# yuz1wan/unified_video_action

Measured on AMD Instinct MI355X. Metric: train samples/sec (video+action step) at 1/2/4/8 MI355X; loss parity, higher is better.
Workload: dtype bf16; 1 GPU; pusht_video: PushT video_model (BASELINE configs[1]); step = frame select+resize -> KL-VAE encode (8 frames) -> mar_base MAR fwd/bwd (N=1024) -> diffusion loss -> backward -> fused AdamW + EMA -> LR step; dropout 0.1; model=UVA mar_base + KL-VAE f16, global_batch=32, seq_len=1024, parallelism=dp1

## Files before the change

unified_video_action_amd/csrc/attention.hip:

```cpp
#include "attention_frag.h"

#define ATT_PRIO_HI() __builtin_amdgcn_s_setprio(1)
#define ATT_PRIO_LO() __builtin_amdgcn_s_setprio(0)
#define AT_LD 80
#define AT_TILE (64 * AT_LD)

__device__ __forceinline__ void stage_load(const bf16* __restrict__ g, long long ld, int row0, bf16x8 (&r)[2]) {
  const int t = threadIdx.x;
  const bf16* base = g + (long long)row0 * ld;
#pragma unroll
  for (int i = 0; i < 2; ++i) {
    const int id = t + i * 256, row = id >> 3, c = (id & 7) * 8;
    r[i] = *(const bf16x8*)(base + (long long)row * ld + c);
  }
}
__device__ __forceinline__ void stage_store(bf16* lds, const bf16x8 (&r)[2]) {
  const int t = threadIdx.x;
#pragma unroll
  for (int i = 0; i < 2; ++i) {
    int id = t + i * 256, row = id >> 3, c = (id & 7) * 8;
    *(bf16x8*)(lds + row * AT_LD + c) = r[i];
  }
}

__device__ __forceinline__ float keep_bfe(float v, uint32_t w, int b) {
  int m;
  asm("v_bfe_i32 %0, %1, %2, 1" : "=v"(m) : "v"(w), "s"(b));
  return __int_as_float(__float_as_int(v) & m);
}
__device__ __forceinline__ float fmax_nc(float a, float b) { return __builtin_amdgcn_fmed3f(a, b, INFINITY); }

constexpr int MASK_TPW = 4;
__device__ __forceinline__ uint32_t shift_in_sign(uint32_t acc, uint32_t t) {
  return __builtin_amdgcn_alignbit(acc, t, 31);
}
__global__ __launch_bounds__(256) void attn_mask_kernel(uint64_t* __restrict__ MQ, uint64_t* __restrict__ MK, int N,
                                                        int nt, long long waves, uint32_t th, uint64_t seed) {
  const long long wv = __builtin_amdgcn_readfirstlane((int)(blockIdx.x * 4u + (threadIdx.x >> 6)));
  if (wv >= waves) return;
  const int L = threadIdx.x & 63;
  const int per_row = (nt + MASK_TPW - 1) / MASK_TPW;
  const int kv0 = (int)(wv % per_row) * MASK_TPW;
  const long long t2 = wv / per_row;
  const int qb = (int)(t2 % nt);
  const long long bh = t2 / nt;
  const int q = qb * 64 + mask_pos(L);
  const uint32_t key = drop_key(seed);
  const uint64_t rowpair = (((uint64_t)bh * N + q) * (uint64_t)N) >> 1;
#pragma unroll 1
  for (int kv = kv0; kv < kv0 + MASK_TPW && kv < nt; ++kv) {
    const uint32_t x0 = drop_first(key, rowpair + (uint64_t)kv * 32);
    uint32_t lo = 0, hi = 0;
#pragma unroll
    for (int P = 31; P >= 0; --P) {
      const uint32_t x = drop_mix(x0 ^ (uint32_t)(mask_pos(2 * P) >> 1));
      const uint32_t t0 = (x & 0xFFFFu) - th, t1 = (x >> 16) - th;
      if (P >= 16) {
        hi = shift_in_sign(shift_in_sign(hi, t1), t0);
      } else {
        lo = shift_in_sign(shift_in_sign(lo, t1), t0);
      }
    }
    lo = ~lo;
    hi = ~hi;
    MQ[((long long)bh * nt + kv) * N + q] = ((uint64_t)hi << 32) | lo;
    {
      const bool up = L & 32;
      const auto r = __builtin_amdgcn_permlane32_swap(up ? lo : hi, up ? lo : hi, false, false);
      const uint32_t o = up ? r[0] : r[1];
      if (up) lo = o; else hi = o;
    }
#define UVA_TSTAGE(J, M)                                                                    \
  {                                                                                         \
    const bool up = L & (J);                                                                \
    const uint32_t sr = up ? 0u : (uint32_t)(J);  \
    const uint32_t km = up ? ~(M) : (M);                                                    \
    const uint32_t rl = (uint32_t)__builtin_amdgcn_ds_swizzle((int)((lo >> sr) & (M)), 0x1F | ((J) << 10)); \
    const uint32_t rh = (uint32_t)__builtin_amdgcn_ds_swizzle((int)((hi >> sr) & (M)), 0x1F | ((J) << 10)); \
    lo = (lo & km) | (rl << sr);                                                            \
    hi = (hi & km) | (rh << sr);                                                            \
  }
    UVA_TSTAGE(16, 0x0000FFFFu)
    UVA_TSTAGE(8, 0x00FF00FFu)
    UVA_TSTAGE(4, 0x0F0F0F0Fu)
    UVA_TSTAGE(2, 0x33333333u)
    UVA_TSTAGE(1, 0x55555555u)
#undef UVA_TSTAGE
    MK[((long long)bh * nt + qb) * N + (long long)kv * 64 + mask_pos(L)] = ((uint64_t)hi << 32) | lo;
  }
}

template <bool DROP, int KT, int OCC>
__global__ __launch_bounds__(256, OCC) void attn_fwd_kernel(const bf16* __restrict__ qkv, bf16* __restrict__ out,
                                                       float* __restrict__ lse2, const uint64_t* __restrict__ MQ,
                                                       int N, int H, float c, float dsc) {
  constexpr int NKT = KT / 16;
  constexpr int NH = KT / 64;
  __shared__ __attribute__((aligned(16))) bf16 sK[2][NH * AT_TILE];
  __shared__ __attribute__((aligned(16))) bf16 sV[2][NH * AT_TILE];
  int bx, bh;
  xcd_grid2(bx, bh);
  const int b = bh / H, h = bh % H;
  const long long ld = 3LL * H * 64;
  const bf16* Qg = qkv + (long long)b * N * ld + h * 64;
  const bf16* Kg = Qg + H * 64;
  const bf16* Vg = Qg + 2 * H * 64;
  const int w = threadIdx.x >> 6, l = threadIdx.x & 63, g = l >> 4, li = l & 15;
  const int q0 = bx * 128 + w * 32;
  const int nkv = N / KT, n64 = N / 64;
  const uint16_t* mq = DROP ? (const uint16_t*)(MQ + (long long)bh * n64 * N) : nullptr;

  bf16x8 qf[2][2];
  uint32_t mw[2][NH], mwn[2][NH];
#pragma unroll
  for (int qt = 0; qt < 2; ++qt) {
    const int row = q0 + qt * 16 + li;
#pragma unroll
    for (int ks = 0; ks < 2; ++ks)
      qf[qt][ks] = row < N ? *(const bf16x8*)(Qg + (long long)row * ld + ks * 32 + 8 * g) : (bf16x8){};
#pragma unroll
    for (int hh = 0; hh < NH; ++hh) {
      mw[qt][hh] = (DROP && row < N) ? mq[((long long)hh * N + row) * 4 + g] : 0u;
      mwn[qt][hh] = 0u;
    }
  }
  float m[2] = {-INFINITY, -INFINITY}, rs[2] = {0.f, 0.f};
  f32x4 o[2][4];
#pragma unroll
  for (int qt = 0; qt < 2; ++qt)
#pragma unroll
    for (int dt = 0; dt < 4; ++dt) o[qt][dt] = (f32x4){0.f, 0.f, 0.f, 0.f};

  bf16x8 rk[NH][2], rv[NH][2];
#pragma unroll
  for (int hh = 0; hh < NH; ++hh) {
    stage_load(Kg, ld, hh * 64, rk[hh]);
    stage_load(Vg, ld, hh * 64, rv[hh]);
  }
#pragma unroll
  for (int hh = 0; hh < NH; ++hh) {
    stage_store(sK[0] + hh * AT_TILE, rk[hh]);
    stage_store(sV[0] + hh * AT_TILE, rv[hh]);
  }
  __syncthreads();
  int cur = 0;
  for (int kv = 0; kv < nkv; ++kv) {
    const bool more = kv + 1 < nkv;
    if (more) {
#pragma unroll
      for (int hh = 0; hh < NH; ++hh) {
        stage_load(Kg, ld, (kv + 1) * KT + hh * 64, rk[hh]);
        stage_load(Vg, ld, (kv + 1) * KT + hh * 64, rv[hh]);
      }
      if (DROP) {
#pragma unroll
        for (int qt = 0; qt < 2; ++qt) {
          const int row = q0 + qt * 16 + li;
#pragma unroll
          for (int hh = 0; hh < NH; ++hh)
            mwn[qt][hh] = row < N ? mq[((long long)((kv + 1) * NH + hh) * N + row) * 4 + g] : 0u;
        }
      }
    }
    const bf16* cK = sK[cur];
    const bf16* cV = sV[cur];
    f32x4 s[NKT][2];
#pragma unroll
    for (int kt = 0; kt < NKT; ++kt)
#pragma unroll
      for (int qt = 0; qt < 2; ++qt) s[kt][qt] = (f32x4){0.f, 0.f, 0.f, 0.f};
    ATT_PRIO_HI();
#pragma unroll
    for (int ks = 0; ks < 2; ++ks) {
#pragma unroll
      for (int kt = 0; kt < NKT; ++kt) {
        const bf16x8 kf = row_frag<AT_LD>(cK, kt * 16, ks);
#pragma unroll
        for (int qt = 0; qt < 2; ++qt) s[kt][qt] = mfma16(kf, qf[qt][ks], s[kt][qt]);
      }
    }
    ATT_PRIO_LO();
    float mx[2];
    bool need = false;
#pragma unroll
    for (int qt = 0; qt < 2; ++qt) {
      float a = fmax_nc(s[0][qt][0], s[0][qt][1]);
#pragma unroll
      for (int kt = 0; kt < NKT; ++kt)
#pragma unroll
        for (int r = (kt == 0 ? 2 : 0); r < 4; ++r) a = fmax_nc(a, s[kt][qt][r]);
      a = quad_max(a);
      mx[qt] = a * c;
      need |= mx[qt] > m[qt] + 8.0f;
    }
    if (__builtin_amdgcn_ballot_w64(need)) {
#pragma unroll
      for (int qt = 0; qt < 2; ++qt) {
        const float mnew = fmaxf(m[qt], mx[qt]);
        const float alpha = exp2_fast(m[qt] - mnew);
        rs[qt] *= alpha;
#pragma unroll
        for (int dt = 0; dt < 4; ++dt) o[qt][dt] *= alpha;
        m[qt] = mnew;
      }
    }
#pragma unroll
    for (int qt = 0; qt < 2; ++qt) {
      const float nm = -m[qt];
      float ps[4] = {0.f, 0.f, 0.f, 0.f};
#pragma unroll
      for (int kt = 0; kt < NKT; ++kt)
#pragma unroll
        for (int r = 0; r < 4; ++r) {
          const float p = exp2_fast(fmaf(s[kt][qt][r], c, nm));
          ps[r] += p;
          s[kt][qt][r] = DROP ? keep_bfe(p, mw[qt][kt >> 2], (kt & 3) * 4 + r) : p;
        }
      rs[qt] += (ps[0] + ps[1]) + (ps[2] + ps[3]);
    }
    ATT_PRIO_HI();
#pragma unroll
    for (int ks = 0; ks < KT / 32; ++ks) {
      bf16x8 pf[2];
#pragma unroll
      for (int qt = 0; qt < 2; ++qt) pf[qt] = pack_pi(s[2 * ks][qt], s[2 * ks + 1][qt]);
#pragma unroll
      for (int dt = 0; dt < 4; ++dt) {
        const bf16x8 vf = tr_frag<AT_LD>(cV, 32 * ks, 32 * ks + 16, dt * 16);
#pragma unroll
        for (int qt = 0; qt < 2; ++qt) o[qt][dt] = mfma16(vf, pf[qt], o[qt][dt]);
      }
    }
    ATT_PRIO_LO();
    if (more) {
#pragma unroll
      for (int hh = 0; hh < NH; ++hh) {
        stage_store(sK[cur ^ 1] + hh * AT_TILE, rk[hh]);
        stage_store(sV[cur ^ 1] + hh * AT_TILE, rv[hh]);
      }
      if (DROP) {
#pragma unroll
        for (int qt = 0; qt < 2; ++qt)
#pragma unroll
          for (int hh = 0; hh < NH; ++hh) mw[qt][hh] = mwn[qt][hh];
      }
    }
    __syncthreads();
    cur ^= 1;
  }
  const long long ldo = (long long)H * 64;
#pragma unroll
  for (int qt = 0; qt < 2; ++qt) {
    float lsum = rs[qt];
    lsum += __shfl_xor(lsum, 16, 64);
    lsum += __shfl_xor(lsum, 32, 64);
    const int q = q0 + qt * 16 + li;
    if (q >= N) continue;
    const float inv = dsc / lsum;
    bf16* orow = out + ((long long)b * N + q) * ldo + h * 64;
#pragma unroll
    for (int dt = 0; dt < 4; ++dt) {
      bf16x4 v = {(bf16)(o[qt][dt][0] * inv), (bf16)(o[qt][dt][1] * inv), (bf16)(o[qt][dt][2] * inv),
                  (bf16)(o[qt][dt][3] * inv)};
      *(bf16x4*)(orow + dt * 16 + 4 * g) = v;
    }
    if (g == 0) lse2[(long long)bh * N + q] = m[qt] + __log2f(lsum);
  }
}

template <bool DROP>
__global__ __launch_bounds__(256, 2) void attn_bwd_dkdv_kernel(const bf16* __restrict__ qkv,
                                                               const bf16* __restrict__ dOs,
                                                               const float* __restrict__ lse2,
                                                               const float* __restrict__ Dvec,
                                                               const uint64_t* __restrict__ MK, bf16* __restrict__ dqkv,
                                                               int N, int H, float scale, float c, float vsc,
                                                               float* __restrict__ cpart) {
  __shared__ __attribute__((aligned(16))) bf16 sQ[2][AT_TILE];
  __shared__ __attribute__((aligned(16))) bf16 sO[2][AT_TILE];
  __shared__ __attribute__((aligned(16))) float sL[2][64];
  __shared__ __attribute__((aligned(16))) float sD[2][64];
  int bx, bh;
  xcd_grid2(bx, bh);
  const int b = bh / H, h = bh % H;
  const long long ld = 3LL * H * 64, ldo = (long long)H * 64;
  const bf16* Qg = qkv + (long long)b * N * ld + h * 64;
  const bf16* Kg = Qg + H * 64;
  const bf16* Vg = Qg + 2 * H * 64;
  const bf16* dOg = dOs + (long long)b * N * ldo + h * 64;
  const float* Lg = lse2 + (long long)bh * N;
  const float* Dg = Dvec + (long long)bh * N;
  const int w = threadIdx.x >> 6, l = threadIdx.x & 63, g = l >> 4, li = l & 15;
  const int k0 = bx * 128 + w * 32;
  const int nq = N / 64;
  const uint16_t* mk = DROP ? (const uint16_t*)(MK + (long long)bh * nq * N) : nullptr;

  bf16x8 kf[2][2], vf[2][2];
  uint32_t mw[2] = {0u, 0u}, mwn[2] = {0u, 0u};
#pragma unroll
  for (int kt = 0; kt < 2; ++kt) {
    const int row = k0 + kt * 16 + li;
    const bool ok = row < N;
#pragma unroll
    for (int ks = 0; ks < 2; ++ks) {
      kf[kt][ks] = ok ? *(const bf16x8*)(Kg + (long long)row * ld + ks * 32 + 8 * g) : (bf16x8){};
      vf[kt][ks] = ok ? *(const bf16x8*)(Vg + (long long)row * ld + ks * 32 + 8 * g) : (bf16x8){};
    }
    if (DROP) mw[kt] = ok ? mk[(long long)row * 4 + g] : 0u;
  }
  f32x4 dv[4][2], dk[4][2];
#pragma unroll
  for (int dt = 0; dt < 4; ++dt)
#pragma unroll
    for (int kt = 0; kt < 2; ++kt) dv[dt][kt] = dk[dt][kt] = (f32x4){0.f, 0.f, 0.f, 0.f};

  bf16x8 rq[2], ro[2];
  stage_load(Qg, ld, 0, rq);
  stage_load(dOg, ldo, 0, ro);
  stage_store(sQ[0], rq);
  stage_store(sO[0], ro);
  if (threadIdx.x < 64) { sL[0][threadIdx.x] = Lg[threadIdx.x]; sD[0][threadIdx.x] = Dg[threadIdx.x]; }
  __syncthreads();
  int cur = 0;
  for (int qi = 0; qi < nq; ++qi) {
    const bool more = qi + 1 < nq;
    float nl = 0.f, nd = 0.f;
    if (more) {
      stage_load(Qg, ld, (qi + 1) * 64, rq);
      stage_load(dOg, ldo, (qi + 1) * 64, ro);
      if (threadIdx.x < 64) { nl = Lg[(qi + 1) * 64 + threadIdx.x]; nd = Dg[(qi + 1) * 64 + threadIdx.x]; }
      if (DROP) {
#pragma unroll
        for (int kt = 0; kt < 2; ++kt) {
          const int row = k0 + kt * 16 + li;
          mwn[kt] = row < N ? mk[((long long)(qi + 1) * N + row) * 4 + g] : 0u;
        }
      }
    }
    f32x4 s[4][2], dp[4][2];
#pragma unroll
    for (int qt = 0; qt < 4; ++qt)
#pragma unroll
      for (int kt = 0; kt < 2; ++kt) s[qt][kt] = dp[qt][kt] = (f32x4){0.f, 0.f, 0.f, 0.f};
#pragma unroll
    for (int ks = 0; ks < 2; ++ks)
#pragma unroll
      for (int qt = 0; qt < 4; ++qt) {
        bf16x8 a = row_frag<AT_LD>(sQ[cur], qt * 16, ks);
        bf16x8 e = row_frag<AT_LD>(sO[cur], qt * 16, ks);
#pragma unroll
        for (int kt = 0; kt < 2; ++kt) {
          s[qt][kt] = mfma16(a, kf[kt][ks], s[qt][kt]);
          dp[qt][kt] = mfma16(e, vf[kt][ks], dp[qt][kt]);
        }
      }
#pragma unroll
    for (int qt = 0; qt < 4; ++qt) {
      const f32x4 Lq = *(const f32x4*)&sL[cur][qt * 16 + 4 * g];
      const f32x4 Dq = *(const f32x4*)&sD[cur][qt * 16 + 4 * g];
#pragma unroll
      for (int r = 0; r < 4; ++r)
#pragma unroll
        for (int kt = 0; kt < 2; ++kt) {
          const float p = exp2_fast(fmaf(s[qt][kt][r], c, -Lq[r]));
          if (DROP) {
            const float pd = keep_bfe(p, mw[kt], qt * 4 + r);
            s[qt][kt][r] = pd;
            dp[qt][kt][r] = fmaf(pd, dp[qt][kt][r], -(p * Dq[r]));
          } else {
            s[qt][kt][r] = p;
            dp[qt][kt][r] = p * (dp[qt][kt][r] - Dq[r]);
          }
        }
    }
#pragma unroll
    for (int ks = 0; ks < 2; ++ks) {
      bf16x8 pb[2], sb[2];
#pragma unroll
      for (int kt = 0; kt < 2; ++kt) {
        pb[kt] = pack_pi(s[2 * ks][kt], s[2 * ks + 1][kt]);
        sb[kt] = pack_pi(dp[2 * ks][kt], dp[2 * ks + 1][kt]);
      }
#pragma unroll
      for (int dt = 0; dt < 4; ++dt) {
        bf16x8 oa = tr_frag<AT_LD>(sO[cur], 32 * ks, 32 * ks + 16, dt * 16);
        bf16x8 qa = tr_frag<AT_LD>(sQ[cur], 32 * ks, 32 * ks + 16, dt * 16);
#pragma unroll
        for (int kt = 0; kt < 2; ++kt) {
          dv[dt][kt] = mfma16(oa, pb[kt], dv[dt][kt]);
          dk[dt][kt] = mfma16(qa, sb[kt], dk[dt][kt]);
        }
      }
    }
    if (more) {
      stage_store(sQ[cur ^ 1], rq);
      stage_store(sO[cur ^ 1], ro);
      if (threadIdx.x < 64) { sL[cur ^ 1][threadIdx.x] = nl; sD[cur ^ 1][threadIdx.x] = nd; }
      if (DROP) { mw[0] = mwn[0]; mw[1] = mwn[1]; }
    }
    lds_barrier();
    cur ^= 1;
  }
  if (cpart) {
    float* red = (float*)&sQ[0][0];
#pragma unroll
    for (int dt = 0; dt < 4; ++dt)
#pragma unroll
      for (int r = 0; r < 4; ++r) {
        float sk = 0.f, sv = 0.f;
#pragma unroll
        for (int kt = 0; kt < 2; ++kt) {
          const bool ok = k0 + kt * 16 + li < N;
          sk += ok ? (float)(bf16)(dk[dt][kt][r] * scale) : 0.f;
          sv += ok ? (float)(bf16)(dv[dt][kt][r] * vsc) : 0.f;
        }
        sk = row16_sum(sk);
        sv = row16_sum(sv);
        if (li == 0) {
          red[w * 128 + dt * 16 + 4 * g + r] = sk;
          red[w * 128 + 64 + dt * 16 + 4 * g + r] = sv;
        }
      }
    __syncthreads();
    if (threadIdx.x < 128) {
      const int t = threadIdx.x;
      const float v = (red[t] + red[128 + t]) + (red[256 + t] + red[384 + t]);
      const long long rowp = (long long)b * gridDim.x + bx;
      cpart[rowp * (3LL * H * 64) + (t < 64 ? H * 64 : 2 * H * 64) + h * 64 + (t & 63)] = v;
    }
  }
#pragma unroll
  for (int kt = 0; kt < 2; ++kt) {
    const int key = k0 + kt * 16 + li;
    if (key >= N) continue;
    bf16* krow = dqkv + ((long long)b * N + key) * ld + H * 64 + h * 64;
    bf16* vrow = krow + H * 64;
#pragma unroll
    for (int dt = 0; dt < 4; ++dt) {
      bf16x4 a = {(bf16)(dk[dt][kt][0] * scale), (bf16)(dk[dt][kt][1] * scale), (bf16)(dk[dt][kt][2] * scale),
                  (bf16)(dk[dt][kt][3] * scale)};
      bf16x4 e = {(bf16)(dv[dt][kt][0] * vsc), (bf16)(dv[dt][kt][1] * vsc), (bf16)(dv[dt][kt][2] * vsc),
                  (bf16)(dv[dt][kt][3] * vsc)};
      *(bf16x4*)(krow + dt * 16 + 4 * g) = a;
      *(bf16x4*)(vrow + dt * 16 + 4 * g) = e;
    }
  }
}

template <bool DROP>
__global__ __launch_bounds__(256, 2) void attn_bwd_dq_kernel(const bf16* __restrict__ qkv,
                                                             const bf16* __restrict__ dOs,
                                                             const bf16* __restrict__ Os,
                                                             const float* __restrict__ lse2,
                                                             float* __restrict__ Dvec,
                                                             const uint64_t* __restrict__ MQ, bf16* __restrict__ dqkv,
                                                             int N, int H, float scale, float c, float dmul,
                                                             float* __restrict__ cpart) {
  __shared__ __attribute__((aligned(16))) bf16 sK[2][AT_TILE];
  __shared__ __attribute__((aligned(16))) bf16 sV[2][AT_TILE];
  int bx, bh;
  xcd_grid2(bx, bh);
  const int b = bh / H, h = bh % H;
  const long long ld = 3LL * H * 64, ldo = (long long)H * 64;
  const bf16* Qg = qkv + (long long)b * N * ld + h * 64;
  const bf16* Kg = Qg + H * 64;
  const bf16* Vg = Qg + 2 * H * 64;
  const bf16* dOg = dOs + (long long)b * N * ldo + h * 64;
  const bf16* Og = Os + (long long)b * N * ldo + h * 64;
  const int w = threadIdx.x >> 6, l = threadIdx.x & 63, g = l >> 4, li = l & 15;
  const int q0 = bx * 128 + w * 32;
  const int nkv = N / 64;
  const uint16_t* mq = DROP ? (const uint16_t*)(MQ + (long long)bh * nkv * N) : nullptr;

  bf16x8 qf[2][2], of[2][2];
  float L[2], Dq[2];
  uint32_t mw[2] = {0u, 0u}, mwn[2] = {0u, 0u};
#pragma unroll
  for (int qt = 0; qt < 2; ++qt) {
    const int row = q0 + qt * 16 + li;
    const bool ok = row < N;
    float dsum = 0.f;
#pragma unroll
    for (int ks = 0; ks < 2; ++ks) {
      qf[qt][ks] = ok ? *(const bf16x8*)(Qg + (long long)row * ld + ks * 32 + 8 * g) : (bf16x8){};
      of[qt][ks] = ok ? *(const bf16x8*)(dOg + (long long)row * ldo + ks * 32 + 8 * g) : (bf16x8){};
      const bf16x8 ov = ok ? *(const bf16x8*)(Og + (long long)row * ldo + ks * 32 + 8 * g) : (bf16x8){};
#pragma unroll
      for (int j = 0; j < 8; ++j) dsum += (float)ov[j] * (float)of[qt][ks][j];
    }
    dsum += __shfl_xor(dsum, 16, 64);
    dsum += __shfl_xor(dsum, 32, 64);
    Dq[qt] = ok ? dsum * dmul : 0.f;
    if (ok && g == 0) Dvec[(long long)bh * N + row] = Dq[qt];
    L[qt] = ok ? lse2[(long long)bh * N + row] : 0.f;
    if (DROP) mw[qt] = ok ? mq[(long long)row * 4 + g] : 0u;
  }
  f32x4 dq[4][2];
#pragma unroll
  for (int dt = 0; dt < 4; ++dt)
#pragma unroll
    for (int qt = 0; qt < 2; ++qt) dq[dt][qt] = (f32x4){0.f, 0.f, 0.f, 0.f};

  bf16x8 rk[2], rv[2];
  stage_load(Kg, ld, 0, rk);
  stage_load(Vg, ld, 0, rv);
  stage_store(sK[0], rk);
  stage_store(sV[0], rv);
  __syncthreads();
  int cur = 0;
  for (int kv = 0; kv < nkv; ++kv) {
    const bool more = kv + 1 < nkv;
    if (more) {
      stage_load(Kg, ld, (kv + 1) * 64, rk);
      stage_load(Vg, ld, (kv + 1) * 64, rv);
      if (DROP) {
#pragma unroll
        for (int qt = 0; qt < 2; ++qt) {
          const int row = q0 + qt * 16 + li;
          mwn[qt] = row < N ? mq[((long long)(kv + 1) * N + row) * 4 + g] : 0u;
        }
      }
    }
    f32x4 s[4][2], dp[4][2];
#pragma unroll
    for (int kt = 0; kt < 4; ++kt)
#pragma unroll
      for (int qt = 0; qt < 2; ++qt) s[kt][qt] = dp[kt][qt] = (f32x4){0.f, 0.f, 0.f, 0.f};
#pragma unroll
    for (int ks = 0; ks < 2; ++ks)
#pragma unroll
      for (int kt = 0; kt < 4; ++kt) {
        const bf16x8 ka = row_frag<AT_LD>(sK[cur], kt * 16, ks);
        const bf16x8 va = row_frag<AT_LD>(sV[cur], kt * 16, ks);
#pragma unroll
        for (int qt = 0; qt < 2; ++qt) {
          s[kt][qt] = mfma16(ka, qf[qt][ks], s[kt][qt]);
          dp[kt][qt] = mfma16(va, of[qt][ks], dp[kt][qt]);
        }
      }
#pragma unroll
    for (int qt = 0; qt < 2; ++qt)
#pragma unroll
      for (int kt = 0; kt < 4; ++kt)
#pragma unroll
        for (int r = 0; r < 4; ++r) {
          const float p = exp2_fast(fmaf(s[kt][qt][r], c, -L[qt]));
          float dpt = dp[kt][qt][r];
          if (DROP) dpt = keep_bfe(dpt, mw[qt], kt * 4 + r);
          s[kt][qt][r] = p * (dpt - Dq[qt]);
        }
#pragma unroll
    for (int ks = 0; ks < 2; ++ks) {
      bf16x8 sb[2];
#pragma unroll
      for (int qt = 0; qt < 2; ++qt) sb[qt] = pack_pi(s[2 * ks][qt], s[2 * ks + 1][qt]);
#pragma unroll
      for (int dt = 0; dt < 4; ++dt) {
        const bf16x8 ka = tr_frag<AT_LD>(sK[cur], 32 * ks, 32 * ks + 16, dt * 16);
#pragma unroll
        for (int qt = 0; qt < 2; ++qt) dq[dt][qt] = mfma16(ka, sb[qt], dq[dt][qt]);
      }
    }
    if (more) {
      stage_store(sK[cur ^ 1], rk);
      stage_store(sV[cur ^ 1], rv);
      if (DROP) { mw[0] = mwn[0]; mw[1] = mwn[1]; }
    }
    lds_barrier();
    cur ^= 1;
  }
  if (cpart) {
    float* red = (float*)&sK[0][0];
#pragma unroll
    for (int dt = 0; dt < 4; ++dt)
#pragma unroll
      for (int r = 0; r < 4; ++r) {
        float sq = 0.f;
#pragma unroll
        for (int qt = 0; qt < 2; ++qt)
          sq += q0 + qt * 16 + li < N ? (float)(bf16)(dq[dt][qt][r] * scale) : 0.f;
        sq = row16_sum(sq);
        if (li == 0) red[w * 64 + dt * 16 + 4 * g + r] = sq;
      }
    __syncthreads();
    if (threadIdx.x < 64) {
      const int t = threadIdx.x;
      const float v = (red[t] + red[64 + t]) + (red[128 + t] + red[192 + t]);
      const long long rowp = (long long)b * gridDim.x + bx;
      cpart[rowp * (3LL * H * 64) + h * 64 + t] = v;
    }
  }
#pragma unroll
  for (int qt = 0; qt < 2; ++qt) {
    const int q = q0 + qt * 16 + li;
    if (q >= N) continue;
    bf16* qrow = dqkv + ((long long)b * N + q) * ld + h * 64;
#pragma unroll
    for (int dt = 0; dt < 4; ++dt) {
      bf16x4 a = {(bf16)(dq[dt][qt][0] * scale), (bf16)(dq[dt][qt][1] * scale), (bf16)(dq[dt][qt][2] * scale),
                  (bf16)(dq[dt][qt][3] * scale)};
      *(bf16x4*)(qrow + dt * 16 + 4 * g) = a;
    }
  }
}

extern "C" long long uva_attn_mask_bytes(int B, int N, int H) {
  return 2LL * B * H * (long long)N * (N / 64) * 8;
}

extern "C" long long uva_attn_bwd_workspace(int B, int N, int H, float drop_p) {
  (void)B; (void)N; (void)H; (void)drop_p;
  return 0;
}

extern "C" int uva_attn_dropmask(void* mask, int B, int N, int H, float drop_p, unsigned long long seed,
                                 hipStream_t s) {
  if (N % 64 != 0 || !(drop_p > 0.f) || mask == nullptr) return (int)hipErrorInvalidValue;
  uint32_t th;
  float ds;
  uva_drop_params(drop_p, &th, &ds);
  const int nt = N / 64;
  uint64_t* MQ = (uint64_t*)mask;
  uint64_t* MK = MQ + (long long)B * H * N * nt;
  const long long waves = (long long)B * H * nt * ((nt + MASK_TPW - 1) / MASK_TPW);
  if (waves > 0x7FFFFFFFLL) return (int)hipErrorInvalidValue;
  attn_mask_kernel<<<dim3((unsigned)((waves + 3) / 4)), 256, 0, s>>>(MQ, MK, N, nt, waves, th, seed);
  UVA_LAUNCH_CHECK();
  return 0;
}

extern "C" int uva_attn_fwd(const void* qkv, void* out, float* lse2, const void* mask, int B, int N, int H,
                            float scale, float drop_p, hipStream_t s) {
  if (N % 64 != 0) return (int)hipErrorInvalidValue;
  const bool drop = drop_p > 0.f;
  if (drop && mask == nullptr) return (int)hipErrorInvalidValue;
  uint32_t th;
  float ds;
  uva_drop_params(drop_p, &th, &ds);
  dim3 grid((N + 127) / 128, B * H);
  const float c = scale * 1.4426950408889634f;
  const uint64_t* MQ = drop ? (const uint64_t*)mask : nullptr;
  if (drop)
    attn_fwd_kernel<true, 64, 3><<<grid, 256, 0, s>>>((const bf16*)qkv, (bf16*)out, lse2, MQ, N, H, c, ds);
  else
    attn_fwd_kernel<false, 64, 3><<<grid, 256, 0, s>>>((const bf16*)qkv, (bf16*)out, lse2, nullptr, N, H, c, 1.0f);
  UVA_LAUNCH_CHECK();
  return 0;
}

static int attn_bwd_launch(const void* qkv, const void* out, const void* dout, const float* lse2, const void* mask,
                           float* Dvec, void* dqkv, int B, int N, int H, float scale, float drop_p, float* cpart,
                           hipStream_t s) {
  if (N % 64 != 0) return (int)hipErrorInvalidValue;
  const bool drop = drop_p > 0.f;
  if (drop && mask == nullptr) return (int)hipErrorInvalidValue;
  uint32_t th;
  float ds;
  uva_drop_params(drop_p, &th, &ds);
  const int nt = N / 64;
  const uint64_t* MQ = (const uint64_t*)mask;
  const uint64_t* MK = drop ? MQ + (long long)B * H * N * nt : nullptr;
  const bf16* dO = (const bf16*)dout;
  dim3 grid((N + 127) / 128, B * H);
  const float c = scale * 1.4426950408889634f;
  const float sk = scale * ds;
  const bf16* O = (const bf16*)out;
  if (drop) {
    attn_bwd_dq_kernel<true><<<grid, 256, 0, s>>>((const bf16*)qkv, dO, O, lse2, Dvec, MQ, (bf16*)dqkv, N, H, sk, c,
                                                  1.0f / ds, cpart);
    attn_bwd_dkdv_kernel<true><<<grid, 256, 0, s>>>((const bf16*)qkv, dO, lse2, Dvec, MK, (bf16*)dqkv, N, H, sk, c, ds,
                                                    cpart);
  } else {
    attn_bwd_dq_kernel<false><<<grid, 256, 0, s>>>((const bf16*)qkv, dO, O, lse2, Dvec, nullptr, (bf16*)dqkv, N, H,
                                                   sk, c, 1.0f, cpart);
    attn_bwd_dkdv_kernel<false><<<grid, 256, 0, s>>>((const bf16*)qkv, dO, lse2, Dvec, nullptr, (bf16*)dqkv, N, H,
                                                     sk, c, ds, cpart);
  }
  UVA_LAUNCH_CHECK();
  return 0;
}

extern "C" int uva_attn_bwd(const void* qkv, const void* out, const void* dout, const float* lse2, const void* mask,
                            float* Dvec, void* dqkv, void* workspace, int B, int N, int H, float scale, float drop_p,
                            hipStream_t s) {
  (void)workspace;
  return attn_bwd_launch(qkv, out, dout, lse2, mask, Dvec, dqkv, B, N, H, scale, drop_p, nullptr, s);
}

int uva_colsum_final_launch(const float* part, int nrows, int cols, float* out, int accum, hipStream_t s);

extern "C" int uva_attn_bwd_bias(const void* qkv, const void* out, const void* dout, const float* lse2,
                                 const void* mask, float* Dvec, void* dqkv, float* dbias, int accum, float* part, int B,
                                 int N, int H, float scale, float drop_p, hipStream_t s) {
  if (!dbias || !part) return (int)hipErrorInvalidValue;
  int r = attn_bwd_launch(qkv, out, dout, lse2, mask, Dvec, dqkv, B, N, H, scale, drop_p, part, s);
  if (r) return r;
  return uva_colsum_final_launch(part, B * ((N + 127) / 128), 3 * H * 64, dbias, accum, s);
}
```

unified_video_action_amd/csrc/attention_frag.h:

```cpp
#pragma once
#include "common.h"

typedef __attribute__((ext_vector_type(2))) __bf16 bf16x2;
typedef __attribute__((ext_vector_type(4))) uint32_t u32x4;

template <int STRIDE>
__device__ __forceinline__ bf16x8 row_frag(const bf16* lds, int row0, int ks) {
  const int l = threadIdx.x & 63;
  return *(const bf16x8*)(lds + (row0 + (l & 15)) * STRIDE + ks * 32 + 8 * (l >> 4));
}

template <int STRIDE>
__device__ __forceinline__ bf16x8 tr_frag(const bf16* lds, int rowA, int rowB, int col0) {
  const int l = threadIdx.x & 63, g = l >> 4, q = (l >> 2) & 3, p = l & 3;
  const bf16* a0 = lds + (rowA + 4 * g + q) * STRIDE + col0 + 4 * p;
  const bf16* a1 = lds + (rowB + 4 * g + q) * STRIDE + col0 + 4 * p;
  s16x4 lo = __builtin_amdgcn_ds_read_tr16_b64_v4i16(LDS_PTR(s16x4, a0));
  s16x4 hi = __builtin_amdgcn_ds_read_tr16_b64_v4i16(LDS_PTR(s16x4, a1));
  s16x8 v = {lo[0], lo[1], lo[2], lo[3], hi[0], hi[1], hi[2], hi[3]};
  return __builtin_bit_cast(bf16x8, v);
}

__device__ __forceinline__ uint32_t cvt_pk_bf16(float lo, float hi) {
  return __builtin_bit_cast(uint32_t, __builtin_convertvector((f32x2){lo, hi}, bf16x2));
}
__device__ __forceinline__ bf16x8 pack_pi(const f32x4& a, const f32x4& b) {
  const u32x4 u = {cvt_pk_bf16(a[0], a[1]), cvt_pk_bf16(a[2], a[3]), cvt_pk_bf16(b[0], b[1]), cvt_pk_bf16(b[2], b[3])};
  return __builtin_bit_cast(bf16x8, u);
}

__device__ __forceinline__ f32x4 mfma16(const bf16x8& a, const bf16x8& b, const f32x4& c) {
  return __builtin_amdgcn_mfma_f32_16x16x32_bf16(a, b, c, 0, 0, 0);
}

__device__ __forceinline__ float exp2_fast(float x) { return __builtin_amdgcn_exp2f(x); }
__device__ __forceinline__ float keep_bit(float v, uint32_t w, int b) {
  return __int_as_float(__float_as_int(v) & __builtin_amdgcn_sbfe(w, b, 1));
}
__device__ __forceinline__ float quad_max(float v) {
  auto r = __builtin_amdgcn_permlane16_swap(__float_as_uint(v), __float_as_uint(v), false, false);
  v = fmaxf(__uint_as_float(r[0]), __uint_as_float(r[1]));
  r = __builtin_amdgcn_permlane32_swap(__float_as_uint(v), __float_as_uint(v), false, false);
  return fmaxf(__uint_as_float(r[0]), __uint_as_float(r[1]));
}
__host__ __device__ constexpr int mask_pos(int k) { return ((k >> 2) & 3) * 16 + (k >> 4) * 4 + (k & 3); }
```

Baseline: 266.8 samples/s.

## Stream attention K/V and Q/dO tiles via direct-to-LDS buffer loads in three-slot ring

Replaces the register-staged double buffer in the attention forward and both backward kernels with buffer_load...lds DMA that writes global tiles straight into a three-slot LDS ring, prefetching two tiles ahead. A new swizzled LDS image layout and matching row and transpose fragment readers replace the padded stride-80 layout. The intent is to remove the VGPR staging and ds_write traffic and to hide more global latency with explicit waitcnt and barrier placement. It raises LDS use, restricts KT to 64, and adds a 32-bit offset range check that can reject very large shapes.

```diff
diff --git a/unified_video_action_amd/csrc/attention.hip b/unified_video_action_amd/csrc/attention.hip
--- a/unified_video_action_amd/csrc/attention.hip
+++ b/unified_video_action_amd/csrc/attention.hip
@@ -1,27 +1,20 @@
 #include "attention_frag.h"
+
+#include <type_traits>
 
 #define ATT_PRIO_HI() __builtin_amdgcn_s_setprio(1)
 #define ATT_PRIO_LO() __builtin_amdgcn_s_setprio(0)
-#define AT_LD 80
-#define AT_TILE (64 * AT_LD)
-
-__device__ __forceinline__ void stage_load(const bf16* __restrict__ g, long long ld, int row0, bf16x8 (&r)[2]) {
-  const int t = threadIdx.x;
-  const bf16* base = g + (long long)row0 * ld;
-#pragma unroll
-  for (int i = 0; i < 2; ++i) {
-    const int id = t + i * 256, row = id >> 3, c = (id & 7) * 8;
-    r[i] = *(const bf16x8*)(base + (long long)row * ld + c);
-  }
-}
-__device__ __forceinline__ void stage_store(bf16* lds, const bf16x8 (&r)[2]) {
-  const int t = threadIdx.x;
-#pragma unroll
-  for (int i = 0; i < 2; ++i) {
-    int id = t + i * 256, row = id >> 3, c = (id & 7) * 8;
-    *(bf16x8*)(lds + row * AT_LD + c) = r[i];
-  }
-}
+#define ATR_WAIT_VM0_LGKM(n) (0x0070 | ((n) << 8))
+#define ATR_SLOT(S) ((S) == 0 ? ring0 : (S) == 1 ? ring1 : ring2)
+#define ATR_SWEEP(step, n)                                               \
+  for (int t_ = 0;;) {                                                   \
+    step(std::integral_constant<int, 0>{}, t_);                          \
+    if (++t_ == (n)) break;                                              \
+    step(std::integral_constant<int, 1>{}, t_);                          \
+    if (++t_ == (n)) break;                                              \
+    step(std::integral_constant<int, 2>{}, t_);                          \
+    if (++t_ == (n)) break;                                              \
+  }
 
 __device__ __forceinline__ float keep_bfe(float v, uint32_t w, int b) {
   int m;
@@ -94,24 +87,26 @@
 __global__ __launch_bounds__(256, OCC) void attn_fwd_kernel(const bf16* __restrict__ qkv, bf16* __restrict__ out,
                                                        float* __restrict__ lse2, const uint64_t* __restrict__ MQ,
                                                        int N, int H, float c, float dsc) {
+  static_assert(KT == 64, "the tile ring streams 64-key tiles");
   constexpr int NKT = KT / 16;
   constexpr int NH = KT / 64;
-  __shared__ __attribute__((aligned(16))) bf16 sK[2][NH * AT_TILE];
-  __shared__ __attribute__((aligned(16))) bf16 sV[2][NH * AT_TILE];
+  constexpr int SLOT = 2 * ATR_TILE;
+  __shared__ __attribute__((aligned(1024))) char ring0[SLOT];
+  __shared__ __attribute__((aligned(1024))) char ring1[SLOT];
+  __shared__ __attribute__((aligned(1024))) char ring2[SLOT];
   int bx, bh;
   xcd_grid2(bx, bh);
   const int b = bh / H, h = bh % H;
   const long long ld = 3LL * H * 64;
   const bf16* Qg = qkv + (long long)b * N * ld + h * 64;
   const bf16* Kg = Qg + H * 64;
-  const bf16* Vg = Qg + 2 * H * 64;
   const int w = threadIdx.x >> 6, l = threadIdx.x & 63, g = l >> 4, li = l & 15;
   const int q0 = bx * 128 + w * 32;
   const int nkv = N / KT, n64 = N / 64;
   const uint16_t* mq = DROP ? (const uint16_t*)(MQ + (long long)bh * n64 * N) : nullptr;
 
   bf16x8 qf[2][2];
-  uint32_t mw[2][NH], mwn[2][NH];
+  uint32_t mw[2][NH];
 #pragma unroll
   for (int qt = 0; qt < 2; ++qt) {
     const int row = q0 + qt * 16 + li;
@@ -121,7 +116,6 @@
 #pragma unroll
     for (int hh = 0; hh < NH; ++hh) {
       mw[qt][hh] = (DROP && row < N) ? mq[((long long)hh * N + row) * 4 + g] : 0u;
-      mwn[qt][hh] = 0u;
     }
   }
   float m[2] = {-INFINITY, -INFINITY}, rs[2] = {0.f, 0.f};
@@ -131,27 +125,29 @@
 #pragma unroll
     for (int dt = 0; dt < 4; ++dt) o[qt][dt] = (f32x4){0.f, 0.f, 0.f, 0.f};
 
-  bf16x8 rk[NH][2], rv[NH][2];
-#pragma unroll
-  for (int hh = 0; hh < NH; ++hh) {
-    stage_load(Kg, ld, hh * 64, rk[hh]);
-    stage_load(Vg, ld, hh * 64, rv[hh]);
-  }
-#pragma unroll
-  for (int hh = 0; hh < NH; ++hh) {
-    stage_store(sK[0] + hh * AT_TILE, rk[hh]);
-    stage_store(sV[0] + hh * AT_TILE, rv[hh]);
-  }
+  const int wu = __builtin_amdgcn_readfirstlane(w);
+  const unsigned ldb = (unsigned)ld * 2u, vofs = (unsigned)H * 128u;
+  const auto rsK = atr_rsrc(Kg, (long long)(N - 1) * ldb + vofs + 128);
+  const unsigned vK = atr_src(l, wu, ldb);
+  auto dma_tile = [&](int t, char* slot) __attribute__((always_inline)) {
+    atr_dma(rsK, slot, wu, vK, (unsigned)t * 64u * ldb, ldb);
+    atr_dma(rsK, slot + ATR_TILE, wu, vK, (unsigned)t * 64u * ldb + vofs, ldb);
+  };
+  dma_tile(0, ring0);
+  if (nkv > 1) dma_tile(1, ring1);
+  __builtin_amdgcn_s_waitcnt(ATR_WAIT_VM0_LGKM(15));
   __syncthreads();
-  int cur = 0;
-  for (int kv = 0; kv < nkv; ++kv) {
+  const int rb = atr_row_base(), tb = atr_tr_base();
+  bf16x8 k0f = atr_row_frag(ring0 + rb, 0, 0);
+  auto step = [&](auto S0c, int kv) __attribute__((always_inline)) {
+    constexpr int S0 = decltype(S0c)::value;
+    char* const r0 = ATR_SLOT(S0);
+    char* const r1 = ATR_SLOT((S0 + 1) % 3);
+    char* const r2 = ATR_SLOT((S0 + 2) % 3);
     const bool more = kv + 1 < nkv;
+    if (kv + 2 < nkv) dma_tile(kv + 2, r2);
+    uint32_t mwn[2][NH] = {};
     if (more) {
-#pragma unroll
-      for (int hh = 0; hh < NH; ++hh) {
-        stage_load(Kg, ld, (kv + 1) * KT + hh * 64, rk[hh]);
-        stage_load(Vg, ld, (kv + 1) * KT + hh * 64, rv[hh]);
-      }
       if (DROP) {
 #pragma unroll
         for (int qt = 0; qt < 2; ++qt) {
@@ -162,8 +158,8 @@
         }
       }
     }
-    const bf16* cK = sK[cur];
-    const bf16* cV = sV[cur];
+    const char* cKr = r0 + rb;
+    const char* cVt = r0 + ATR_TILE + tb;
     f32x4 s[NKT][2];
 #pragma unroll
     for (int kt = 0; kt < NKT; ++kt)
@@ -174,7 +170,7 @@
     for (int ks = 0; ks < 2; ++ks) {
 #pragma unroll
       for (int kt = 0; kt < NKT; ++kt) {
-        const bf16x8 kf = row_frag<AT_LD>(cK, kt * 16, ks);
+        const bf16x8 kf = (ks | kt) ? atr_row_frag(cKr, kt * 16, ks) : k0f;
 #pragma unroll
         for (int qt = 0; qt < 2; ++qt) s[kt][qt] = mfma16(kf, qf[qt][ks], s[kt][qt]);
       }
@@ -226,28 +222,25 @@
       for (int qt = 0; qt < 2; ++qt) pf[qt] = pack_pi(s[2 * ks][qt], s[2 * ks + 1][qt]);
 #pragma unroll
       for (int dt = 0; dt < 4; ++dt) {
-        const bf16x8 vf = tr_frag<AT_LD>(cV, 32 * ks, 32 * ks + 16, dt * 16);
+        const bf16x8 vf = atr_tr_frag(cVt, 32 * ks, 32 * ks + 16, dt * 16);
 #pragma unroll
         for (int qt = 0; qt < 2; ++qt) o[qt][dt] = mfma16(vf, pf[qt], o[qt][dt]);
       }
     }
     ATT_PRIO_LO();
-    if (more) {
-#pragma unroll
-      for (int hh = 0; hh < NH; ++hh) {
-        stage_store(sK[cur ^ 1] + hh * AT_TILE, rk[hh]);
-        stage_store(sV[cur ^ 1] + hh * AT_TILE, rv[hh]);
-      }
-      if (DROP) {
-#pragma unroll
-        for (int qt = 0; qt < 2; ++qt)
-#pragma unroll
-          for (int hh = 0; hh < NH; ++hh) mw[qt][hh] = mwn[qt][hh];
-      }
-    }
-    __syncthreads();
-    cur ^= 1;
-  }
+    if (DROP) {
+#pragma unroll
+      for (int qt = 0; qt < 2; ++qt)
+#pragma unroll
+        for (int hh = 0; hh < NH; ++hh) mw[qt][hh] = mwn[qt][hh];
+    }
+    __builtin_amdgcn_sched_barrier(0);
+    k0f = atr_row_frag(r1 + rb, 0, 0);
+    __builtin_amdgcn_s_waitcnt(ATR_WAIT_VM0_LGKM(1));
+    __builtin_amdgcn_s_barrier();
+    __builtin_amdgcn_sched_barrier(0);
+  };
+  ATR_SWEEP(step, nkv);
   const long long ldo = (long long)H * 64;
 #pragma unroll
   for (int qt = 0; qt < 2; ++qt) {
@@ -276,8 +269,10 @@
                                                                const uint64_t* __restrict__ MK, bf16* __restrict__ dqkv,
                                                                int N, int H, float scale, float c, float vsc,
                                                                float* __restrict__ cpart) {
-  __shared__ __attribute__((aligned(16))) bf16 sQ[2][AT_TILE];
-  __shared__ __attribute__((aligned(16))) bf16 sO[2][AT_TILE];
+  constexpr int SLOT = 2 * ATR_TILE;
+  __shared__ __attribute__((aligned(1024))) char ring0[SLOT];
+  __shared__ __attribute__((aligned(1024))) char ring1[SLOT];
+  __shared__ __attribute__((aligned(1024))) char ring2[SLOT];
   __shared__ __attribute__((aligned(16))) float sL[2][64];
   __shared__ __attribute__((aligned(16))) float sD[2][64];
   int bx, bh;
@@ -296,7 +291,7 @@
   const uint16_t* mk = DROP ? (const uint16_t*)(MK + (long long)bh * nq * N) : nullptr;
 
   bf16x8 kf[2][2], vf[2][2];
-  uint32_t mw[2] = {0u, 0u}, mwn[2] = {0u, 0u};
+  uint32_t mw[2] = {0u, 0u};
 #pragma unroll
   for (int kt = 0; kt < 2; ++kt) {
     const int row = k0 + kt * 16 + li;
@@ -314,20 +309,37 @@
 #pragma unroll
     for (int kt = 0; kt < 2; ++kt) dv[dt][kt] = dk[dt][kt] = (f32x4){0.f, 0.f, 0.f, 0.f};
 
-  bf16x8 rq[2], ro[2];
-  stage_load(Qg, ld, 0, rq);
-  stage_load(dOg, ldo, 0, ro);
-  stage_store(sQ[0], rq);
-  stage_store(sO[0], ro);
+  const int wu = __builtin_amdgcn_readfirstlane(w);
+  const unsigned ldb = (unsigned)ld * 2u, ldob = (unsigned)ldo * 2u;
+  const auto rsQ = atr_rsrc(Qg, (long long)(N - 1) * ldb + 128);
+  const auto rsO = atr_rsrc(dOg, (long long)(N - 1) * ldob + 128);
+  const unsigned vQ = atr_src(l, wu, ldb), vO = atr_src(l, wu, ldob);
+  auto dma_tile = [&](int t, char* slot) __attribute__((always_inline)) {
+    atr_dma(rsQ, slot, wu, vQ, (unsigned)t * 64u * ldb, ldb);
+    atr_dma(rsO, slot + ATR_TILE, wu, vO, (unsigned)t * 64u * ldob, ldob);
+  };
+  dma_tile(0, ring0);
+  if (nq > 1) dma_tile(1, ring1);
   if (threadIdx.x < 64) { sL[0][threadIdx.x] = Lg[threadIdx.x]; sD[0][threadIdx.x] = Dg[threadIdx.x]; }
+  __builtin_amdgcn_s_waitcnt(ATR_WAIT_VM0_LGKM(15));
   __syncthreads();
+  const int rb = atr_row_base(), tb = atr_tr_base();
+  bf16x8 a0 = atr_row_frag(ring0 + rb, 0, 0), e0 = atr_row_frag(ring0 + ATR_TILE + rb, 0, 0);
   int cur = 0;
-  for (int qi = 0; qi < nq; ++qi) {
+  auto step = [&](auto S0c, int qi) __attribute__((always_inline)) {
+    constexpr int S0 = decltype(S0c)::value;
+    char* const r0 = ATR_SLOT(S0);
+    char* const r1 = ATR_SLOT((S0 + 1) % 3);
+    char* const r2 = ATR_SLOT((S0 + 2) % 3);
     const bool more = qi + 1 < nq;
     float nl = 0.f, nd = 0.f;
+    uint32_t mwn[2] = {0u, 0u};
+    if (qi + 2 < nq) dma_tile(qi + 2, r2);
+    const char* cQr = r0 + rb;
+    const char* cOr = cQr + ATR_TILE;
+    const char* cQt = r0 + tb;
+    const char* cOt = cQt + ATR_TILE;
     if (more) {
-      stage_load(Qg, ld, (qi + 1) * 64, rq);
-      stage_load(dOg, ldo, (qi + 1) * 64, ro);
       if (threadIdx.x < 64) { nl = Lg[(qi + 1) * 64 + threadIdx.x]; nd = Dg[(qi + 1) * 64 + threadIdx.x]; }
       if (DROP) {
 #pragma unroll
@@ -346,8 +358,8 @@
     for (int ks = 0; ks < 2; ++ks)
 #pragma unroll
       for (int qt = 0; qt < 4; ++qt) {
-        bf16x8 a = row_frag<AT_LD>(sQ[cur], qt * 16, ks);
-        bf16x8 e = row_frag<AT_LD>(sO[cur], qt * 16, ks);
+        bf16x8 a = (ks | qt) ? atr_row_frag(cQr, qt * 16, ks) : a0;
+        bf16x8 e = (ks | qt) ? atr_row_frag(cOr, qt * 16, ks) : e0;
 #pragma unroll
         for (int kt = 0; kt < 2; ++kt) {
           s[qt][kt] = mfma16(a, kf[kt][ks], s[qt][kt]);
@@ -383,8 +395,8 @@
       }
 #pragma unroll
       for (int dt = 0; dt < 4; ++dt) {
-        bf16x8 oa = tr_frag<AT_LD>(sO[cur], 32 * ks, 32 * ks + 16, dt * 16);
-        bf16x8 qa = tr_frag<AT_LD>(sQ[cur], 32 * ks, 32 * ks + 16, dt * 16);
+        bf16x8 oa = atr_tr_frag(cOt, 32 * ks, 32 * ks + 16, dt * 16);
+        bf16x8 qa = atr_tr_frag(cQt, 32 * ks, 32 * ks + 16, dt * 16);
 #pragma unroll
         for (int kt = 0; kt < 2; ++kt) {
           dv[dt][kt] = mfma16(oa, pb[kt], dv[dt][kt]);
@@ -393,16 +405,20 @@
       }
     }
     if (more) {
-      stage_store(sQ[cur ^ 1], rq);
-      stage_store(sO[cur ^ 1], ro);
       if (threadIdx.x < 64) { sL[cur ^ 1][threadIdx.x] = nl; sD[cur ^ 1][threadIdx.x] = nd; }
-      if (DROP) { mw[0] = mwn[0]; mw[1] = mwn[1]; }
-    }
-    lds_barrier();
+    }
+    if (DROP) { mw[0] = mwn[0]; mw[1] = mwn[1]; }
+    __builtin_amdgcn_sched_barrier(0);
+    a0 = atr_row_frag(r1 + rb, 0, 0);
+    e0 = atr_row_frag(r1 + ATR_TILE + rb, 0, 0);
+    __builtin_amdgcn_s_waitcnt(ATR_WAIT_VM0_LGKM(2));
+    __builtin_amdgcn_s_barrier();
+    __builtin_amdgcn_sched_barrier(0);
     cur ^= 1;
-  }
+  };
+  ATR_SWEEP(step, nq);
   if (cpart) {
-    float* red = (float*)&sQ[0][0];
+    float* red = (float*)ring0;
 #pragma unroll
     for (int dt = 0; dt < 4; ++dt)
 #pragma unroll
@@ -456,15 +472,16 @@
                                                              const uint64_t* __restrict__ MQ, bf16* __restrict__ dqkv,
                                                              int N, int H, float scale, float c, float dmul,
                                                              float* __restrict__ cpart) {
-  __shared__ __attribute__((aligned(16))) bf16 sK[2][AT_TILE];
-  __shared__ __attribute__((aligned(16))) bf16 sV[2][AT_TILE];
+  constexpr int SLOT = 2 * ATR_TILE;
+  __shared__ __attribute__((aligned(1024))) char ring0[SLOT];
+  __shared__ __attribute__((aligned(1024))) char ring1[SLOT];
+  __shared__ __attribute__((aligned(1024))) char ring2[SLOT];
   int bx, bh;
   xcd_grid2(bx, bh);
   const int b = bh / H, h = bh % H;
   const long long ld = 3LL * H * 64, ldo = (long long)H * 64;
   const bf16* Qg = qkv + (long long)b * N * ld + h * 64;
   const bf16* Kg = Qg + H * 64;
-  const bf16* Vg = Qg + 2 * H * 64;
   const bf16* dOg = dOs + (long long)b * N * ldo + h * 64;
   const bf16* Og = Os + (long long)b * N * ldo + h * 64;
   const int w = threadIdx.x >> 6, l = threadIdx.x & 63, g = l >> 4, li = l & 15;
@@ -474,7 +491,7 @@
 
   bf16x8 qf[2][2], of[2][2];
   float L[2], Dq[2];
-  uint32_t mw[2] = {0u, 0u}, mwn[2] = {0u, 0u};
+  uint32_t mw[2] = {0u, 0u};
 #pragma unroll
   for (int qt = 0; qt < 2; ++qt) {
     const int row = q0 + qt * 16 + li;
@@ -501,18 +518,32 @@
 #pragma unroll
     for (int qt = 0; qt < 2; ++qt) dq[dt][qt] = (f32x4){0.f, 0.f, 0.f, 0.f};
 
-  bf16x8 rk[2], rv[2];
-  stage_load(Kg, ld, 0, rk);
-  stage_load(Vg, ld, 0, rv);
-  stage_store(sK[0], rk);
-  stage_store(sV[0], rv);
+  const int wu = __builtin_amdgcn_readfirstlane(w);
+  const unsigned ldb = (unsigned)ld * 2u, vofs = (unsigned)H * 128u;
+  const auto rsK = atr_rsrc(Kg, (long long)(N - 1) * ldb + vofs + 128);
+  const unsigned vK = atr_src(l, wu, ldb);
+  auto dma_tile = [&](int t, char* slot) __attribute__((always_inline)) {
+    atr_dma(rsK, slot, wu, vK, (unsigned)t * 64u * ldb, ldb);
+    atr_dma(rsK, slot + ATR_TILE, wu, vK, (unsigned)t * 64u * ldb + vofs, ldb);
+  };
+  dma_tile(0, ring0);
+  if (nkv > 1) dma_tile(1, ring1);
+  __builtin_amdgcn_s_waitcnt(ATR_WAIT_VM0_LGKM(15));
   __syncthreads();
-  int cur = 0;
-  for (int kv = 0; kv < nkv; ++kv) {
+  const int rb = atr_row_base(), tb = atr_tr_base();
+  bf16x8 k0f = atr_row_frag(ring0 + rb, 0, 0), v0f = atr_row_frag(ring0 + ATR_TILE + rb, 0, 0);
+  auto step = [&](auto S0c, int kv) __attribute__((always_inline)) {
+    constexpr int S0 = decltype(S0c)::value;
+    char* const r0 = ATR_SLOT(S0);
+    char* const r1 = ATR_SLOT((S0 + 1) % 3);
+    char* const r2 = ATR_SLOT((S0 + 2) % 3);
     const bool more = kv + 1 < nkv;
+    uint32_t mwn[2] = {0u, 0u};
+    if (kv + 2 < nkv) dma_tile(kv + 2, r2);
+    const char* cKr = r0 + rb;
+    const char* cVr = cKr + ATR_TILE;
+    const char* cKt = r0 + tb;
     if (more) {
-      stage_load(Kg, ld, (kv + 1) * 64, rk);
-      stage_load(Vg, ld, (kv + 1) * 64, rv);
       if (DROP) {
 #pragma unroll
         for (int qt = 0; qt < 2; ++qt) {
@@ -530,8 +561,8 @@
     for (int ks = 0; ks < 2; ++ks)
 #pragma unroll
       for (int kt = 0; kt < 4; ++kt) {
-        const bf16x8 ka = row_frag<AT_LD>(sK[cur], kt * 16, ks);
-        const bf16x8 va = row_frag<AT_LD>(sV[cur], kt * 16, ks);
+        const bf16x8 ka = (ks | kt) ? atr_row_frag(cKr, kt * 16, ks) : k0f;
+        const bf16x8 va = (ks | kt) ? atr_row_frag(cVr, kt * 16, ks) : v0f;
 #pragma unroll
         for (int qt = 0; qt < 2; ++qt) {
           s[kt][qt] = mfma16(ka, qf[qt][ks], s[kt][qt]);
@@ -556,21 +587,22 @@
       for (int qt = 0; qt < 2; ++qt) sb[qt] = pack_pi(s[2 * ks][qt], s[2 * ks + 1][qt]);
 #pragma unroll
       for (int dt = 0; dt < 4; ++dt) {
-        const bf16x8 ka = tr_frag<AT_LD>(sK[cur], 32 * ks, 32 * ks + 16, dt * 16);
+        const bf16x8 ka = atr_tr_frag(cKt, 32 * ks, 32 * ks + 16, dt * 16);
 #pragma unroll
         for (int qt = 0; qt < 2; ++qt) dq[dt][qt] = mfma16(ka, sb[qt], dq[dt][qt]);
       }
     }
-    if (more) {
-      stage_store(sK[cur ^ 1], rk);
-      stage_store(sV[cur ^ 1], rv);
-      if (DROP) { mw[0] = mwn[0]; mw[1] = mwn[1]; }
-    }
-    lds_barrier();
-    cur ^= 1;
-  }
+    if (DROP) { mw[0] = mwn[0]; mw[1] = mwn[1]; }
+    __builtin_amdgcn_sched_barrier(0);
+    k0f = atr_row_frag(r1 + rb, 0, 0);
+    v0f = atr_row_frag(r1 + ATR_TILE + rb, 0, 0);
+    __builtin_amdgcn_s_waitcnt(ATR_WAIT_VM0_LGKM(2));
+    __builtin_amdgcn_s_barrier();
+    __builtin_amdgcn_sched_barrier(0);
+  };
+  ATR_SWEEP(step, nkv);
   if (cpart) {
-    float* red = (float*)&sK[0][0];
+    float* red = (float*)ring0;
 #pragma unroll
     for (int dt = 0; dt < 4; ++dt)
 #pragma unroll
@@ -603,6 +635,8 @@
     }
   }
 }
+
+static bool atr_range_ok(int N, int H) { return N > 0 && H > 0 && (double)N * 3.0 * H * 128.0 < 2147483648.0; }
 
 extern "C" long long uva_attn_mask_bytes(int B, int N, int H) {
   return 2LL * B * H * (long long)N * (N / 64) * 8;
@@ -631,7 +665,7 @@
 
 extern "C" int uva_attn_fwd(const void* qkv, void* out, float* lse2, const void* mask, int B, int N, int H,
                             float scale, float drop_p, hipStream_t s) {
-  if (N % 64 != 0) return (int)hipErrorInvalidValue;
+  if (N % 64 != 0 || !atr_range_ok(N, H)) return (int)hipErrorInvalidValue;
   const bool drop = drop_p > 0.f;
   if (drop && mask == nullptr) return (int)hipErrorInvalidValue;
   uint32_t th;
@@ -651,7 +685,7 @@
 static int attn_bwd_launch(const void* qkv, const void* out, const void* dout, const float* lse2, const void* mask,
                            float* Dvec, void* dqkv, int B, int N, int H, float scale, float drop_p, float* cpart,
                            hipStream_t s) {
-  if (N % 64 != 0) return (int)hipErrorInvalidValue;
+  if (N % 64 != 0 || !atr_range_ok(N, H)) return (int)hipErrorInvalidValue;
   const bool drop = drop_p > 0.f;
   if (drop && mask == nullptr) return (int)hipErrorInvalidValue;
   uint32_t th;
diff --git a/unified_video_action_amd/csrc/attention_frag.h b/unified_video_action_amd/csrc/attention_frag.h
--- a/unified_video_action_amd/csrc/attention_frag.h
+++ b/unified_video_action_amd/csrc/attention_frag.h
@@ -15,6 +15,42 @@
   const int l = threadIdx.x & 63, g = l >> 4, q = (l >> 2) & 3, p = l & 3;
   const bf16* a0 = lds + (rowA + 4 * g + q) * STRIDE + col0 + 4 * p;
   const bf16* a1 = lds + (rowB + 4 * g + q) * STRIDE + col0 + 4 * p;
+  s16x4 lo = __builtin_amdgcn_ds_read_tr16_b64_v4i16(LDS_PTR(s16x4, a0));
+  s16x4 hi = __builtin_amdgcn_ds_read_tr16_b64_v4i16(LDS_PTR(s16x4, a1));
+  s16x8 v = {lo[0], lo[1], lo[2], lo[3], hi[0], hi[1], hi[2], hi[3]};
+  return __builtin_bit_cast(bf16x8, v);
+}
+
+constexpr int ATR_TILE = 8192;
+constexpr int ATR_QUARTER = 2048;
+constexpr int ATR_PIECES = 8;
+constexpr int ATR_SLOTS = 3;
+
+__device__ __forceinline__ unsigned atr_src(int lane, int wave, unsigned ldb) {
+  return (unsigned)(lane >> 1) * ldb + (unsigned)(wave * 32 + (lane & 1) * 16);
+}
+__device__ __forceinline__ __amdgpu_buffer_rsrc_t atr_rsrc(const void* p, long long bytes) {
+  return __builtin_amdgcn_make_buffer_rsrc((void*)p, 0, (int)(unsigned)(bytes < 0xffffffffLL ? bytes : 0xffffffffLL),
+                                           0x00020000);
+}
+__device__ __forceinline__ void atr_dma(__amdgpu_buffer_rsrc_t rs, char* img, int wave, unsigned voff, unsigned soff,
+                                        unsigned ldb) {
+  __builtin_amdgcn_raw_ptr_buffer_load_lds(rs, (__attribute__((address_space(3))) void*)(img + wave * 2048), 16,
+                                           (int)voff, (int)soff, 0, 0);
+  __builtin_amdgcn_raw_ptr_buffer_load_lds(rs, (__attribute__((address_space(3))) void*)(img + wave * 2048 + 1024), 16,
+                                           (int)voff, (int)(soff + 32u * ldb), 0, 0);
+}
+__device__ __forceinline__ int atr_row_base() {
+  const int l = threadIdx.x & 63, g = l >> 4;
+  return (g >> 1) * ATR_QUARTER + (l & 15) * 32 + (g & 1) * 16;
+}
+__device__ __forceinline__ int atr_tr_base() { return 8 * (threadIdx.x & 63); }
+__device__ __forceinline__ bf16x8 atr_row_frag(const char* img_rb, int row0, int ks) {
+  return *(const bf16x8*)(img_rb + ks * 2 * ATR_QUARTER + row0 * 32);
+}
+__device__ __forceinline__ bf16x8 atr_tr_frag(const char* img_tb, int rowA, int rowB, int col0) {
+  const char* a0 = img_tb + (col0 >> 4) * ATR_QUARTER + rowA * 32;
+  const char* a1 = img_tb + (col0 >> 4) * ATR_QUARTER + rowB * 32;
   s16x4 lo = __builtin_amdgcn_ds_read_tr16_b64_v4i16(LDS_PTR(s16x4, a0));
   s16x4 hi = __builtin_amdgcn_ds_read_tr16_b64_v4i16(LDS_PTR(s16x4, a1));
   s16x8 v = {lo[0], lo[1], lo[2], lo[3], hi[0], hi[1], hi[2], hi[3]};
```

Measured after the change: 266.3 samples/s. Within noise of the previous version (-0.2%).
